# acappemin/Video-to-Audio-and-Piano-RP

Measured on AMD Instinct MI355X. Metric: mel-frames/sec (10s VGGSound shape, 32-step CFM, CFG 2.0), higher is better.
Workload: dtype bf16x3; 1 GPU; BASELINE.json configs[1]: 1 clip(s)/GPU x 750 latent frames x 128 ch, 32-point sway grid = 31 CFG evaluations (62 DiT forwards), T5 context 16 tokens, V2A zero roll; clips_per_gpu=1, global_clips=1, parallelism=clip-sharded x1, 1 all-gather, hipgraph=True, schedule=three streams, side_streams=True, cascade_passes=1

## Files before the change

### video-to-audio-and-piano-rp_amd/csrc/gemm_8phase.hip

```cpp
#include "gemm_common.h"

namespace {

#if defined(V2A_GEMM_PROBE) && defined(V2A_8PH_SKIP)
constexpr int kSkip = V2A_8PH_SKIP;
#else
constexpr int kSkip = 0;
#endif

template <int EPI, typename OutT, int MODE, bool SPLIT>
__global__ __launch_bounds__(512) void gemm_bf16_8ph_kernel(GemmParams p) {
  constexpr bool STAGGER = MODE != 2;
  constexpr int BM = 256, BN = 256, WM = 128, WN = 64, TM = 8, TN = 4;
  constexpr int HALF = 128 * 128;
  constexpr int BUF = 4 * HALF;
  static_assert(!is_glu(EPI) || (TN % 2 == 0), "GEGLU / SWIGLU need value/gate tile pairs");
  extern __shared__ __attribute__((aligned(16))) char smem_raw[];

  const int tid = threadIdx.x;
  const int lane = tid & 63;
  const int wave = __builtin_amdgcn_readfirstlane(tid >> 6);
  const int wr = wave >> 2, wc = wave & 3;
  const int lr = lane & 15, lq = lane >> 4;

  int tm, tn;
  tile_of_block(p, blockIdx.x, tm, tn);
  const int m0 = tm * BM, n0 = tn * BN;

  f32x4 acc[TM][TN];
#pragma unroll
  for (int i = 0; i < TM; ++i)
#pragma unroll
    for (int j = 0; j < TN; ++j) acc[i][j] = f32x4{0.f, 0.f, 0.f, 0.f};

  const int srow = lane >> 3;
  const int schunk = (lane & 7) ^ srow;
  const uint32_t schunk_b = (uint32_t)((SPLIT ? schunk & 3 : schunk) << 4);
  const bool slo = SPLIT && schunk >= 4;
  const int kl = SPLIT ? p.s3_kl : 0;
  uint32_t woff[2][2];
#pragma unroll
  for (int s = 0; s < 2; ++s)
#pragma unroll
    for (int i = 0; i < 2; ++i) {
      const int r = 8 * (wave + 8 * i) + srow;
      const int wrw = n0 + 64 * (r >> 5) + (r & 31) + 32 * s;
      woff[s][i] = (uint32_t)(((int64_t)(wrw < p.N ? wrw : p.N - 1) * p.ldw) * 2) + schunk_b + (slo ? (uint32_t)kl * 2 : 0u);
    }
  const char* wbase = reinterpret_cast<const char*>(p.w);
  constexpr int KS = SPLIT ? 32 : 64;
  constexpr int KSH = SPLIT ? 5 : 6;
  const int nk = p.K / KS;

  const int nseg = p.nseg;
  const int64_t a0 = (int64_t)p.a[0];
  const int64_t da1 = nseg > 1 ? (int64_t)p.a[1] - a0 : 0, da2 = nseg > 2 ? (int64_t)p.a[2] - (int64_t)p.a[1] : 0;
  const int32_t ldb0 = (int32_t)(p.lda[0] * 2);
  const int32_t dl1 = nseg > 1 ? (int32_t)(p.lda[1] * 2) - ldb0 : 0, dl2 = nseg > 2 ? (int32_t)((p.lda[2] - p.lda[1]) * 2) : 0;
  const int kend0 = nseg > 1 ? p.kend[0] : 0x7fffffff, kend1 = nseg > 2 ? p.kend[1] : 0x7fffffff;
  const int dk2 = nseg > 2 ? p.kend[1] - p.kend[0] : 0;
  const int sb0 = SPLIT ? (int)(2 * p.alo[0]) : 0;
  const int dsb1 = SPLIT && nseg > 1 ? (int)(2 * p.alo[1]) - sb0 : 0;
  const int dsb2 = SPLIT && nseg > 2 ? (int)(2 * p.alo[2]) - (sb0 + dsb1) : 0;
  const char* aptr[2];
  int aleft[2] = {0, 0};
  uint32_t aoff[2][2];
  auto a_setup = [&](int s, int kt) {
    const int k0 = kt * KS;
    const bool s1 = k0 >= kend0, s2 = k0 >= kend1;
    const int kbeg = (s1 ? kend0 : 0) + (s2 ? dk2 : 0);
    aptr[s] = reinterpret_cast<const char*>(a0 + (s1 ? da1 : 0) + (s2 ? da2 : 0)) + (int64_t)(k0 - kbeg) * 2;
    const uint32_t ldb = (uint32_t)(ldb0 + (s1 ? dl1 : 0) + (s2 ? dl2 : 0));
    const uint32_t lo = slo ? (uint32_t)(sb0 + (s1 ? dsb1 : 0) + (s2 ? dsb2 : 0)) : 0u;
    const int kstop = min(p.K, s2 ? 0x7fffffff : (s1 ? kend1 : kend0));
    aleft[s] = (kstop - k0) >> KSH;
#pragma unroll
    for (int i = 0; i < 2; ++i) {
      const int r = 8 * (wave + 8 * i) + srow;
      const int ar = m0 + r + ((r >= 64) ? 64 : 0) + 64 * s;
      aoff[s][i] = (uint32_t)(ar < p.M ? ar : p.M - 1) * ldb + schunk_b + lo;
    }
  };
  auto stage_a = [&](int s, int kt, int buf) {
    if (aleft[s] == 0) a_setup(s, kt);
    char* dst = smem_raw + buf * BUF + s * HALF;
#pragma unroll
    for (int i = 0; i < 2; ++i)
      __builtin_amdgcn_global_load_lds((const __attribute__((address_space(1))) void*)(aptr[s] + aoff[s][i]),
                                       (__attribute__((address_space(3))) void*)(dst + (wave + 8 * i) * 1024), 16, 0, 0);
    aptr[s] += 2 * KS;
    --aleft[s];
  };
  const char* wptr = wbase;
  int wleft = 0;
  auto stage_b = [&](int kt, int buf) {
    if (wleft == 0) {
      wptr = wbase + (int64_t)kt * (2 * KS);
      wleft = nk - kt;
    }
#pragma unroll
    for (int s = 0; s < 2; ++s) {
      char* dst = smem_raw + buf * BUF + (2 + s) * HALF;
#pragma unroll
      for (int i = 0; i < 2; ++i) {
        uint32_t wo = woff[s][i];
        asm volatile("" : "+v"(wo));
        __builtin_amdgcn_global_load_lds((const __attribute__((address_space(1))) void*)(wptr + wo),
                                         (__attribute__((address_space(3))) void*)(dst + (wave + 8 * i) * 1024), 16, 0, 0);
      }
    }
    wptr += 2 * KS;
    --wleft;
  };

  const int a_frag_off = (64 * wr + lr) * 128;
  const int b_frag_off = (32 * wc + lr) * 128;
  const int ch0 = ((0 + lq) ^ (lr & 7)) << 4, ch1 = ((4 + lq) ^ (lr & 7)) << 4;
  bf16x8 af[4][2], bf0[2][2], bf1[2][2];
  auto read_a = [&](int s, int buf) {
    const char* base = smem_raw + buf * BUF + s * HALF + a_frag_off;
#pragma unroll
    for (int i = 0; i < 4; ++i) {
      af[i][0] = *reinterpret_cast<const bf16x8*>(base + i * 2048 + ch0);
      af[i][1] = *reinterpret_cast<const bf16x8*>(base + i * 2048 + ch1);
    }
  };
  auto read_b = [&](int s, int buf, bf16x8 (&bf)[2][2]) {
    const char* base = smem_raw + buf * BUF + (2 + s) * HALF + b_frag_off;
#pragma unroll
    for (int j = 0; j < 2; ++j) {
      bf[j][0] = *reinterpret_cast<const bf16x8*>(base + j * 2048 + ch0);
      bf[j][1] = *reinterpret_cast<const bf16x8*>(base + j * 2048 + ch1);
    }
  };
  const int rows_valid = (p.dbg & 512) ? 256 : p.M - m0;
  const bool need0 = wr * 128 < rows_valid, need1 = wr * 128 + 64 < rows_valid;
  auto quadrant = [&](auto sa_c, auto sb_c, const bf16x8 (&bf)[2][2]) {
    constexpr int SA = decltype(sa_c)::value, SB = decltype(sb_c)::value;
    if (!(SA == 0 ? need0 : need1)) return;
    __builtin_amdgcn_s_setprio(1);
    if constexpr (SPLIT) {
#pragma unroll
      for (int t = 0; t < 3; ++t)
#pragma unroll
        for (int i = 0; i < 4; ++i)
#pragma unroll
          for (int j = 0; j < 2; ++j)
            acc[4 * SA + i][2 * SB + j] =
                __builtin_amdgcn_mfma_f32_16x16x32_bf16(af[i][t == 0 ? 1 : 0], bf[j][t == 1 ? 1 : 0], acc[4 * SA + i][2 * SB + j], 0, 0, 0);
    } else {
#pragma unroll
      for (int kk = 0; kk < 2; ++kk)
#pragma unroll
        for (int i = 0; i < 4; ++i)
#pragma unroll
          for (int j = 0; j < 2; ++j)
            acc[4 * SA + i][2 * SB + j] = __builtin_amdgcn_mfma_f32_16x16x32_bf16(af[i][kk], bf[j][kk], acc[4 * SA + i][2 * SB + j], 0, 0, 0);
    }
    __builtin_amdgcn_s_setprio(0);
  };
  using I0 = std::integral_constant<int, 0>;
  using I1 = std::integral_constant<int, 1>;

  float* rs_lds = reinterpret_cast<float*>(smem_raw + 2 * BUF);
  const bool scaled = p.rssq != nullptr && p.vec_epi;
  RowScaleLoad rsl;
  if (scaled && tid < 256) rowscale_load(p, m0 + tid, rsl);
  stage_a(0, 0, 0);
  stage_b(0, 0);
  stage_a(1, 0, 0);
  if (nk > 1) {
    stage_a(0, 1, 1);
    stage_b(1, 1);
    if (scaled && tid < 256) rs_lds[tid] = rowscale_finish(p, rsl);
    asm volatile("s_waitcnt vmcnt(6)" ::: "memory");
  } else {
    if (scaled && tid < 256) rs_lds[tid] = rowscale_finish(p, rsl);
    asm volatile("s_waitcnt vmcnt(0)" ::: "memory");
  }
  __builtin_amdgcn_s_barrier();
  if constexpr (STAGGER) {
    if (wr == 1) __builtin_amdgcn_s_barrier();
  }

  auto ktile = [&](auto buf_c, int t) {
    constexpr int B = decltype(buf_c)::value;
    if (!(kSkip & 4) || t == 0) read_a(0, B);
    if (!(kSkip & 1) || t == 0) read_b(0, B, bf0);
    __builtin_amdgcn_sched_barrier(0);
    __builtin_amdgcn_s_barrier();
    quadrant(I0{}, I0{}, bf0);
    __builtin_amdgcn_sched_barrier(0);
    __builtin_amdgcn_s_barrier();
    if (!(kSkip & 1) || t == 0) read_b(1, B, bf1);
    if (t + 1 < nk && !(kSkip & 8)) stage_a(1, t + 1, B ^ 1);
    __builtin_amdgcn_sched_barrier(0);
    __builtin_amdgcn_s_barrier();
    quadrant(I0{}, I1{}, bf1);
    __builtin_amdgcn_sched_barrier(0);
    __builtin_amdgcn_s_barrier();
    if (!(kSkip & 4) || t == 0) read_a(1, B);
    if (t + 2 < nk && !(kSkip & 8)) stage_a(0, t + 2, B);
    __builtin_amdgcn_sched_barrier(0);
    __builtin_amdgcn_s_barrier();
    quadrant(I1{}, I1{}, bf1);
    __builtin_amdgcn_sched_barrier(0);
    __builtin_amdgcn_s_barrier();
    if (t + 2 < nk) {
      if (!(kSkip & 2)) stage_b(t + 2, B);
      asm volatile("s_waitcnt vmcnt(6)" ::: "memory");
    } else {
      asm volatile("s_waitcnt vmcnt(0)" ::: "memory");
    }
    __builtin_amdgcn_sched_barrier(0);
    __builtin_amdgcn_s_barrier();
    quadrant(I1{}, I0{}, bf0);
    __builtin_amdgcn_sched_barrier(0);
    __builtin_amdgcn_s_barrier();
  };
  for (int t = 0; t < nk; t += 2) {
    ktile(I0{}, t);
    if (t + 1 < nk) ktile(I1{}, t + 1);
  }
  if constexpr (STAGGER) {
    if (wr == 0) __builtin_amdgcn_s_barrier();
  }
  if (p.vec_epi) {
    static_assert(8 * 16 * (WN + 4) * 4 <= 2 * BUF, "epilogue slabs must fit in the ring memory");
    float* tile = reinterpret_cast<float*>(smem_raw) + wave * (16 * (WN + 4));
    EpiPrefetch<EPI, TM, WN, false> pf;
    gemm_epilogue_lds<EPI, OutT, TM, TN, WM, WN, false>(p, acc, tile, m0 + wr * WM, n0 + wc * WN, lane, pf, scaled ? rs_lds + wr * WM : nullptr);
  } else {
    gemm_epilogue<EPI, OutT, TM, TN, WM, WN>(p, acc, m0, n0, wr, wc, lr, lq);
  }
}

template <int EPI, typename OutT>
int launch_8ph(const GemmParams& p_in, hipStream_t s) {
  GemmParams p = p_in;
  v2a_detail::fill_tile_map(p, 256, 256);
  constexpr size_t smem = 2 * 4 * 128 * 128 + 256 * 4;
  const int tiles = ((p.M + 255) / 256) * ((p.N + 255) / 256);
  const int mode = v2a_detail::g_gemm_tuning.use_8phase;
  auto go = [&](auto kern) -> int {
    static std::atomic<uint64_t> lds_set{0};
    if (int rc = v2a_enable_lds(reinterpret_cast<const void*>(kern), smem, lds_set, "v2a_gemm(8-phase)")) return rc;
    hipLaunchKernelGGL(kern, dim3(tiles), dim3(512), smem, s, p);
    return 0;
  };
  int rc;
  if (p.s3_kl != 0) {
    if (mode == 2) rc = go(gemm_bf16_8ph_kernel<EPI, OutT, 2, true>);
    else rc = go(gemm_bf16_8ph_kernel<EPI, OutT, 1, true>);
  } else if constexpr (EPI == V2A_EPI_GELU || EPI == V2A_EPI_SWIGLU) {
    return v2a_fail(V2A_ERR_ARG, "v2a_gemm(8-phase): GELU / SWIGLU need split operands");
  } else {
    if (mode == 2) rc = go(gemm_bf16_8ph_kernel<EPI, OutT, 2, false>);
    else rc = go(gemm_bf16_8ph_kernel<EPI, OutT, 1, false>);
  }
  if (rc) return rc;
  return v2a_check_launch("v2a_gemm(8-phase)");
}

}

int v2a_detail::launch_gemm_8phase(const GemmParams& p, int epilogue, int out_dtype, hipStream_t s) {
  const bool out_f32 = out_dtype == V2A_F32;
  switch (epilogue) {
    case V2A_EPI_STORE:
      return out_f32 ? launch_8ph<V2A_EPI_STORE, float>(p, s) : launch_8ph<V2A_EPI_STORE, bf16_t>(p, s);
    case V2A_EPI_GEGLU:
      return out_f32 ? launch_8ph<V2A_EPI_GEGLU, float>(p, s) : launch_8ph<V2A_EPI_GEGLU, bf16_t>(p, s);
    case V2A_EPI_GELU:
      if (p.s3_kl) return out_f32 ? launch_8ph<V2A_EPI_GELU, float>(p, s) : launch_8ph<V2A_EPI_GELU, bf16_t>(p, s);
      break;
    case V2A_EPI_SWIGLU:
      if (p.s3_kl) return out_f32 ? launch_8ph<V2A_EPI_SWIGLU, float>(p, s) : launch_8ph<V2A_EPI_SWIGLU, bf16_t>(p, s);
      break;
    case V2A_EPI_RESID:
      if (out_f32) return launch_8ph<V2A_EPI_RESID, float>(p, s);
      break;
    case V2A_EPI_GATE_RESID:
      if (out_f32) return launch_8ph<V2A_EPI_GATE_RESID, float>(p, s);
      break;
  }
  return v2a_fail(V2A_ERR_ARG, "v2a_gemm(8-phase): unsupported epilogue %d / out_dtype %d", epilogue, out_dtype);
}
```

### video-to-audio-and-piano-rp_amd/csrc/gemm_common.h

```cpp
#pragma once
#include "v2a_common.h"
#include <stdlib.h>
#include <type_traits>

namespace v2a_detail {

struct GemmParams {
  const void* a[3];
  int64_t lda[3];
  int32_t kend[3];
  int32_t nseg;
  const void* w;
  int64_t ldw;
  const float* bias;
  int32_t M, N, K;
  void* out;
  int64_t ldo;
  bf16_t* out2;
  int64_t ldo2;
  const float* resid;
  int64_t ldr;
  const float* gate;
  const int32_t* step;
  int64_t gss, gbs;
  int32_t rpb;
  const float* rope;
  int32_t rope_cols, rope_pos_off;
  int32_t vec_epi;
  int32_t relu;
  const int32_t* a_rowoff;
  const int32_t* a_koff;
  const int32_t* o_rowoff;
  int32_t krot;
  const float* ngam;
  int64_t ngss, ngbs;
  int32_t nsw_row, nsw_off;
  float* ssq;
  int64_t ssq_ld;
  const float* rssq;
  int64_t rssq_ld;
  int32_t rssq_parts;
  float rnorm;
  int32_t xcd_gm, xcd_gn;
  struct Rect { int32_t m_lo, n_lo, cnt, hm; float rcp; } rect[8];
  int32_t nrect, tiles_m, tiles_n;
  int32_t out2_split, out_split;
  int64_t alo[3];
  int64_t out2_lo;
  int32_t s3_kl;
  int32_t dbg;
};

struct GemmTuning {
  int force_tile;
  int krot;
  int use_8phase;
  int min_tiles_8phase;
  int xcd_grid;
  int dbg;
};
extern GemmTuning g_gemm_tuning;
extern int g_attn_one_group_from;
extern int g_dwconv_rows_per_wave;
extern int g_probe_dbg;
extern int g_dwconv_stream;

int launch_gemm_8phase(const GemmParams& p, int epilogue, int out_dtype, hipStream_t stream);

inline void fill_tile_map(GemmParams& p, int BM, int BN) {
  p.tiles_m = (p.M + BM - 1) / BM;
  p.tiles_n = (p.N + BN - 1) / BN;
  const int gm = p.xcd_gm, gn = p.xcd_gn;
  p.nrect = gm * gn;
  for (int r = 0; r < p.nrect; ++r) {
    const int xm = r / gn, xn = r % gn;
    const int m_lo = xm * p.tiles_m / gm, m_hi = (xm + 1) * p.tiles_m / gm;
    const int n_lo = xn * p.tiles_n / gn, n_hi = (xn + 1) * p.tiles_n / gn;
    const int hm = m_hi - m_lo;
    p.rect[r].m_lo = m_lo;
    p.rect[r].n_lo = n_lo;
    p.rect[r].cnt = hm * (n_hi - n_lo);
    p.rect[r].hm = hm > 0 ? hm : 1;
    p.rect[r].rcp = 1.0f / (float)(hm > 0 ? hm : 1);
  }
}

}

namespace {

using v2a_detail::GemmParams;

__device__ __forceinline__ void tile_of_index(const GemmParams& p, int L, int& tm, int& tn) {
  tm = tn = 0;
#pragma unroll
  for (int r = 0; r < 8; ++r) {
    if (r < p.nrect) {
      const int cnt = p.rect[r].cnt;
      if (L >= 0 && L < cnt) {
        const int hm = p.rect[r].hm;
        int q = (int)((float)L * p.rect[r].rcp);
        int rem = L - q * hm;
        if (rem < 0) { --q; rem += hm; }
        else if (rem >= hm) { ++q; rem -= hm; }
        tn = p.rect[r].n_lo + q;
        tm = p.rect[r].m_lo + rem;
      }
      L -= cnt;
    }
  }
}
__device__ __forceinline__ void tile_of_block(const GemmParams& p, int bid, int& tm, int& tn) {
  const int nwg = p.tiles_m * p.tiles_n;
  const int q = nwg >> 3, r = nwg & 7, xcd = bid & 7;
  const int L = (xcd < r ? xcd * (q + 1) : r * (q + 1) + (xcd - r) * q) + (bid >> 3);
  tile_of_index(p, L, tm, tn);
}

__host__ __device__ constexpr bool is_glu(int epi) { return epi == V2A_EPI_GEGLU || epi == V2A_EPI_SWIGLU; }
template <int EPI, bool FAST> __device__ __forceinline__ float glu_act(float g) {
  if constexpr (EPI == V2A_EPI_SWIGLU) return FAST ? silu_f(g) : silu_exact_f(g);
  else return FAST ? gelu_fast_f(g) : gelu_erf_f(g);
}

template <typename T> struct TileCfg;
template <> struct TileCfg<bf16_t> {
  static constexpr int BK = 64;
  static constexpr int LDS_ROW = 64;
};
template <> struct TileCfg<float> {
  static constexpr int BK = 16;
  static constexpr int LDS_ROW = 20;
};

template <int ROWS, bool SRC_F32> struct StageBf16 {
  static constexpr int N = ROWS / 32;
  bf16x8 r[N];
  __device__ __forceinline__ void load(const void* base, int64_t ld, int row0, int rows_total, int k0, int tid) {
    const int chunk = tid & 7;
#pragma unroll
    for (int i = 0; i < N; ++i) {
      int row = row0 + (tid >> 3) + 32 * i;
      row = row < rows_total ? row : rows_total - 1;
      if constexpr (SRC_F32) {
        const float* p = reinterpret_cast<const float*>(base) + (int64_t)row * ld + k0 + chunk * 8;
        f32x4 lo = *reinterpret_cast<const f32x4*>(p);
        f32x4 hi = *reinterpret_cast<const f32x4*>(p + 4);
        bf16x8 v;
#pragma unroll
        for (int j = 0; j < 4; ++j) {
          v[j] = (bf16_t)lo[j];
          v[4 + j] = (bf16_t)hi[j];
        }
        r[i] = v;
      } else {
        const bf16_t* p = reinterpret_cast<const bf16_t*>(base) + (int64_t)row * ld + k0 + chunk * 8;
        r[i] = *reinterpret_cast<const bf16x8*>(p);
      }
    }
  }
  __device__ __forceinline__ void store(bf16_t* lds, int tid) const {
    const int chunk = tid & 7;
#pragma unroll
    for (int i = 0; i < N; ++i) {
      int row = (tid >> 3) + 32 * i;
      *reinterpret_cast<bf16x8*>(lds + row * 64 + ((chunk ^ (row & 7)) << 3)) = r[i];
    }
  }
};

template <int ROWS> struct StageF32 {
  static constexpr int N = ROWS / 64;
  f32x4 r[N];
  __device__ __forceinline__ void load(const void* base, int64_t ld, int row0, int rows_total, int k0, int tid) {
    const int c4 = tid & 3;
#pragma unroll
    for (int i = 0; i < N; ++i) {
      int row = row0 + (tid >> 2) + 64 * i;
      row = row < rows_total ? row : rows_total - 1;
      const float* p = reinterpret_cast<const float*>(base) + (int64_t)row * ld + k0 + c4 * 4;
      r[i] = *reinterpret_cast<const f32x4*>(p);
    }
  }
  __device__ __forceinline__ void store(float* lds, int tid) const {
    const int c4 = tid & 3;
#pragma unroll
    for (int i = 0; i < N; ++i) {
      int row = (tid >> 2) + 64 * i;
      *reinterpret_cast<f32x4*>(lds + row * 20 + c4 * 4) = r[i];
    }
  }
};

template <typename T, bool A_F32, int ROWS> struct StageSel;
template <bool A_F32, int ROWS> struct StageSel<bf16_t, A_F32, ROWS> { using type = StageBf16<ROWS, A_F32>; };
template <bool A_F32, int ROWS> struct StageSel<float, A_F32, ROWS> { using type = StageF32<ROWS>; };

template <int EPI, typename OutT, int TM, int TN, int WM, int WN>
__device__ __forceinline__ void gemm_epilogue(const GemmParams& p, f32x4 (&acc)[TM][TN], int m0, int n0, int wm, int wn,
                                              int lr, int lq) {
  OutT* out = reinterpret_cast<OutT*>(p.out);
#pragma unroll
  for (int i = 0; i < TM; ++i) {
#pragma unroll
    for (int jj = 0; jj < 4; ++jj) {
      const int m = m0 + wm * WM + i * 16 + lq * 4 + jj;
      if (m >= p.M) continue;
      const float* gvec = nullptr;
      if constexpr (EPI == V2A_EPI_GATE_RESID) gvec = step_vec(p.gate, p.step, p.gss, p.gbs, p.gbs ? m / p.rpb : 0);
      if constexpr (is_glu(EPI)) {
#pragma unroll
        for (int j = 0; j < TN; j += 2) {
          const int n = n0 + wn * WN + j * 16 + lr;
          if (n >= p.N) continue;
          float v = acc[i][j][jj], g = acc[i][j + 1][jj];
          if (p.bias) { v += p.bias[n]; g += p.bias[n + 16]; }
          const int oc = ((n0 + wn * WN) >> 1) + (j >> 1) * 16 + lr;
          const float ge = glu_act<EPI, sizeof(OutT) == 2>(g);
          out[(int64_t)m * p.ldo + oc] = from_f32<OutT>(v * ge);
        }
      } else {
#pragma unroll
        for (int j = 0; j < TN; ++j) {
          const int n = n0 + wn * WN + j * 16 + lr;
          if (n >= p.N) continue;
          float v = acc[i][j][jj];
          if (p.bias) v += p.bias[n];
          if constexpr (EPI == V2A_EPI_SIGMOID) v = sigmoid_f(v);
          if constexpr (EPI == V2A_EPI_GELU) v = gelu_erf_f(v);
          if constexpr (EPI == V2A_EPI_RESID) v += p.resid[(int64_t)m * p.ldr + n];
          if constexpr (EPI == V2A_EPI_GATE_RESID) v = p.resid[(int64_t)m * p.ldr + n] + gvec[n] * v;
          if (p.relu) v = fmaxf(v, 0.f);
          out[(int64_t)m * p.ldo + n] = from_f32<OutT>(v);
          if constexpr (sizeof(OutT) == 4) {
            if (p.out2) p.out2[(int64_t)m * p.ldo2 + n] = (bf16_t)v;
          }
        }
      }
    }
  }
}


template <int EPI, int TM, int WN, bool ON> struct EpiPrefetch {
  static constexpr int LPR = WN / 4, RPI = 64 / LPR, RPS = 16 / RPI;
  static constexpr bool RES = ON && (EPI == V2A_EPI_RESID || EPI == V2A_EPI_GATE_RESID);
  static constexpr bool GATE = ON && EPI == V2A_EPI_GATE_RESID;
  f32x4 rs[RES ? TM : 1][RES ? RPS : 1];
  f32x4 gt[GATE ? TM : 1][GATE ? RPS : 1];
  static constexpr bool SCAT = RES && !GATE;
  int32_t ro[SCAT ? TM : 1][SCAT ? RPS : 1];
  static constexpr bool ROPE = ON && EPI == V2A_EPI_STORE;
  f32x4 cs[ROPE ? TM : 1][ROPE ? RPS : 1];
  __device__ __forceinline__ void load(const GemmParams& p, int m_base, int n_base, int lane) {
    if constexpr (ROPE) {
      const int c4 = (lane % LPR) * 4, r0 = lane / LPR;
      const int n = n_base + c4;
      if (p.rope && n < p.rope_cols) {
#pragma unroll
        for (int i = 0; i < TM; ++i)
#pragma unroll
          for (int q = 0; q < RPS; ++q) {
            int m = m_base + i * 16 + r0 + q * RPI;
            m = m < p.M ? m : p.M - 1;
            const int pos = p.rope_pos_off + m % p.rpb;
            cs[i][q] = *reinterpret_cast<const f32x4*>(p.rope + ((int64_t)pos * 32 + ((n & 63) >> 1)) * 2);
          }
      }
    }
    if constexpr (RES) {
      const int c4 = (lane % LPR) * 4, r0 = lane / LPR;
      const int n = n_base + c4;
      const int M = p.M;
      const bool full = n + 3 < p.N;
      const bool has_res = p.resid != nullptr, has_gate = p.gate != nullptr;
      const float* resid = p.resid + n;
      const int64_t ldr = p.ldr;
      const int32_t* orow = SCAT ? p.o_rowoff : nullptr;
      if constexpr (SCAT) {
        if (orow) {
#pragma unroll
          for (int i = 0; i < TM; ++i)
#pragma unroll
            for (int q = 0; q < RPS; ++q) {
              int m = m_base + i * 16 + r0 + q * RPI;
              m = m < M ? m : M - 1;
              ro[i][q] = orow[m];
            }
        }
      }
#pragma unroll
      for (int i = 0; i < TM; ++i)
#pragma unroll
        for (int q = 0; q < RPS; ++q) {
          const int m = m_base + i * 16 + r0 + q * RPI;
          if (m < M && full) {
            int64_t off = (int64_t)m * ldr;
            if constexpr (SCAT) { if (orow) off = ro[i][q]; }
            rs[i][q] = has_res ? *reinterpret_cast<const f32x4*>(resid + off) : f32x4{0.f, 0.f, 0.f, 0.f};
            if constexpr (GATE) gt[i][q] = has_gate ? *reinterpret_cast<const f32x4*>(step_vec(p.gate, p.step, p.gss, p.gbs, p.gbs ? m / p.rpb : 0) + n) : f32x4{1.f, 1.f, 1.f, 1.f};
          }
        }
    }
  }
};

constexpr int kRowSsqMax = 40;
struct RowScaleLoad {
  f32x4 v[kRowSsqMax / 4];
};
__device__ __forceinline__ void rowscale_load(const GemmParams& p, int m, RowScaleLoad& r) {
  m = m < p.M ? m : p.M - 1;
  const float* q = p.rssq + (int64_t)m * p.rssq_ld;
#pragma unroll
  for (int k = 0; k < kRowSsqMax / 4; ++k) {
    r.v[k] = f32x4{0.f, 0.f, 0.f, 0.f};
    if (4 * k < p.rssq_parts) r.v[k] = *reinterpret_cast<const f32x4*>(q + 4 * k);
  }
}
__device__ __forceinline__ float rowscale_finish(const GemmParams& p, const RowScaleLoad& r) {
  float s = 0.f;
#pragma unroll
  for (int k = 0; k < kRowSsqMax / 4; ++k) s += (r.v[k][0] + r.v[k][1]) + (r.v[k][2] + r.v[k][3]);
  return p.rnorm / fmaxf(sqrtf(s), 1e-12f);
}

__device__ __forceinline__ void rope_rotate4(f32x4& v, const f32x4& cs) {
  const float a0 = v[0], b0 = v[1], a1 = v[2], b1 = v[3];
  v[0] = fmaf(a0, cs[0], -(b0 * cs[1]));
  v[1] = fmaf(b0, cs[0], a0 * cs[1]);
  v[2] = fmaf(a1, cs[2], -(b1 * cs[3]));
  v[3] = fmaf(b1, cs[2], a1 * cs[3]);
}

__device__ __forceinline__ void row_pos(int p0, int d, int rpb, bool multi, int& pos, int& nb) {
  pos = p0 + d;
  nb = 0;
  if (pos >= rpb) { pos -= rpb; nb = 1; }
  if (multi) {
    while (pos >= rpb) { pos -= rpb; ++nb; }
  }
}

template <int EPI, bool PF> constexpr bool epi_pipelined() { return !PF && (EPI == V2A_EPI_STORE || EPI == V2A_EPI_RESID || EPI == V2A_EPI_GATE_RESID); }

template <int EPI, typename OutT, int TM, int TN, int WM, int WN, bool PF, bool ALL>
__device__ __forceinline__ void gemm_epilogue_lds_impl(const GemmParams& p, f32x4 (&acc)[TM][TN], float* tile, int m_base, int n_base, int lane,
                                                       const EpiPrefetch<EPI, TM, WN, PF>& pf, const float* rs_row) {
  constexpr int LD = WN + 4;
  const int lr = lane & 15, lq = lane >> 4;
  OutT* out = reinterpret_cast<OutT*>(p.out);
  const int M = p.M, N = p.N;
  const bool relu = p.relu != 0;
  const int32_t* orow = ALL ? nullptr : p.o_rowoff;
  const int64_t ldo = p.ldo, ldr = p.ldr, ldo2 = p.ldo2;
  bf16_t* out2 = p.out2;
  const float* resid = p.resid;
  const float* bias = p.bias;
  constexpr int LPRX = (is_glu(EPI) ? WN / 2 : WN) / 4;
  constexpr int RPSX = 16 / (64 / LPRX);
  constexpr bool RESF = EPI == V2A_EPI_RESID || EPI == V2A_EPI_GATE_RESID;
  constexpr bool GAMF = RESF && sizeof(OutT) == 4;
  constexpr bool PIPE = epi_pipelined<EPI, PF>();
  static_assert(PIPE || !ALL, "the unpredicated form belongs to the pipeline");
  constexpr int LPRV = WN / 4, RPIV = 64 / LPRV, RPSV = 16 / RPIV;
  const int c4v = (lane % LPRV) * 4, r0v = lane / LPRV;
  const int nv = n_base + c4v;
  const bool fullv = nv + 3 < N;
  const bool scaled = rs_row != nullptr;
  const bool geglu_wide = is_glu(EPI) && sizeof(OutT) == 2 && (WN / 2) % 32 == 0 && ((uintptr_t)p.out & 15) == 0 && (p.ldo & 7) == 0 &&
                          ((p.N >> 1) & 7) == 0 && !(p.dbg & 128);

  f32x4 bb[is_glu(EPI) ? 4 : 1];
#pragma unroll
  for (int k = 0; k < (is_glu(EPI) ? 4 : 1); ++k) bb[k] = f32x4{0.f, 0.f, 0.f, 0.f};
  if constexpr (is_glu(EPI)) {
    if (geglu_wide) {
      const int c8 = (lane % (WN / 16)) * 8;
      const int n = n_base + (c8 >> 4) * 32 + (c8 & 15);
      if (bias && n < N) {
        bb[0] = *reinterpret_cast<const f32x4*>(bias + n);
        bb[1] = *reinterpret_cast<const f32x4*>(bias + n + 4);
        bb[2] = *reinterpret_cast<const f32x4*>(bias + n + 16);
        bb[3] = *reinterpret_cast<const f32x4*>(bias + n + 20);
      }
    } else {
      const int c4 = (lane % (WN / 8)) * 4;
      const int n = n_base + (c4 >> 4) * 32 + (c4 & 15);
      if (bias && n < N) {
        bb[0] = *reinterpret_cast<const f32x4*>(bias + n);
        bb[2] = *reinterpret_cast<const f32x4*>(bias + n + 16);
      }
    }
  } else {
    if (bias && fullv) bb[0] = *reinterpret_cast<const f32x4*>(bias + nv);
  }
  const float* gate_b = nullptr;
  const float* ngam_b = nullptr;
  if constexpr (RESF) {
    const int64_t stepv = p.step ? (int64_t)p.step[0] : 0;
    if (p.gate) gate_b = p.gate + stepv * p.gss;
    if (p.ngam) ngam_b = p.ngam + stepv * p.ngss;
  }
  const int rpb = p.rpb;
  const bool rope_on = PIPE && EPI == V2A_EPI_STORE && p.rope != nullptr && n_base < p.rope_cols;
  static_assert(64 % WN == 0 || EPI != V2A_EPI_STORE || PF, "a wave's columns lie in one 64-column head");
  const bool gate_pb = PIPE && EPI == V2A_EPI_GATE_RESID && gate_b != nullptr && p.gbs != 0;
  const bool gam_on = GAMF && out2 != nullptr && ngam_b != nullptr;
  const bool gam_pb = gam_on && p.ngbs != 0;
  int b0 = 0, p0 = 0;
  bool onebatch = true, twobatch = true;
  if (rope_on || gate_pb || (PIPE && gam_pb)) {
    const int mb = __builtin_amdgcn_readfirstlane(m_base);
    b0 = mb / rpb;
    p0 = mb - b0 * rpb;
    const int last = p0 + ((mb + WM < M ? mb + WM : M) - 1 - mb);
    onebatch = last < rpb;
    twobatch = last < 2 * rpb;
  }
  const int m_sw = m_base - p0 + rpb;
  const bool multi = rpb < WM;
  const bool gate_row = gate_pb && !twobatch, gam_row = gam_pb && !(PIPE && twobatch);
  const bool gate_two = gate_pb && !onebatch && !gate_row, gam_two = PIPE && gam_pb && !onebatch && !gam_row;
  f32x4 gmA = {1.f, 1.f, 1.f, 1.f}, gmB = gmA, gmC = gmA, gmD = gmA, gt1 = gmA, gt2 = gmA;
  if constexpr (GAMF) {
    if (gam_on && !gam_row && fullv && m_base < M) {
      const float* gb = ngam_b + (gam_pb ? (int64_t)b0 * p.ngbs : 0) + nv;
      gmA = *reinterpret_cast<const f32x4*>(gb);
      gmB = *reinterpret_cast<const f32x4*>(gb + p.nsw_off);
      if constexpr (PIPE) {
        if (gam_two) {
          gmC = *reinterpret_cast<const f32x4*>(gb + p.ngbs);
          gmD = *reinterpret_cast<const f32x4*>(gb + p.ngbs + p.nsw_off);
        }
      }
    }
  }
  if constexpr (PIPE && EPI == V2A_EPI_GATE_RESID) {
    if (gate_b && !gate_row && fullv && m_base < M) {
      const float* gp = gate_b + (gate_pb ? (int64_t)b0 * p.gbs : 0) + nv;
      gt1 = *reinterpret_cast<const f32x4*>(gp);
      if (gate_two) gt2 = *reinterpret_cast<const f32x4*>(gp + p.gbs);
    }
  }
  float rsc[PIPE ? 1 : TM][PIPE ? 1 : RPSX];
  if constexpr (!PIPE) {
    if (scaled) {
#pragma unroll
      for (int i = 0; i < TM; ++i)
#pragma unroll
        for (int q = 0; q < RPSX; ++q) rsc[i][q] = rs_row[i * 16 + lane / LPRX + q * (64 / LPRX)];
    }
  }

  f32x4 q_a[PIPE ? 2 : 1][PIPE ? RPSV : 1];
  {
#pragma unroll
    for (int i = -1; i < TM; ++i) {
      if (!ALL && m_base + (i < 0 ? 0 : i) * 16 >= M) break;
      if constexpr (PIPE) {
        if (i + 1 < TM && (ALL || m_base + (i + 1) * 16 < M)) {
#pragma unroll
          for (int q = 0; q < RPSV; ++q) {
            const int m = m_base + (i + 1) * 16 + r0v + q * RPIV;
            const bool ok = ALL || (m < M && fullv);
            if constexpr (EPI == V2A_EPI_STORE) {
              if (rope_on && ok) {
                int pos, nb;
                row_pos(p0, m - m_base, rpb, multi, pos, nb);
                q_a[(i + 1) & 1][q] = *reinterpret_cast<const f32x4*>(p.rope + ((int64_t)(p.rope_pos_off + pos) * 32 + ((nv & 63) >> 1)) * 2);
              }
            }
            if constexpr (RESF) {
              if (ok) {
                int64_t o_res = (int64_t)m * ldr;
                if constexpr (EPI == V2A_EPI_RESID) { if (orow) o_res = orow[m]; }
                q_a[(i + 1) & 1][q] = *reinterpret_cast<const f32x4*>(resid + o_res + nv);
              }
            }
          }
        }
        __builtin_amdgcn_sched_barrier(0);
      }
      if (i < 0) continue;
      if constexpr (PIPE) __builtin_amdgcn_sched_barrier(0);
#pragma unroll
      for (int j = 0; j < TN; ++j)
#pragma unroll
        for (int jj = 0; jj < 4; ++jj) tile[(lq * 4 + jj) * LD + j * 16 + lr] = acc[i][j][jj];
      if (i == 0) {
#pragma unroll
        for (int k = 0; k < (is_glu(EPI) ? 4 : 1); ++k) asm volatile("" : "+v"(bb[k]));
        if constexpr (GAMF) asm volatile("" : "+v"(gmA), "+v"(gmB), "+v"(gmC), "+v"(gmD));
        if constexpr (PIPE && EPI == V2A_EPI_GATE_RESID) asm volatile("" : "+v"(gt1), "+v"(gt2));
      }
      if constexpr (is_glu(EPI) && sizeof(OutT) == 2 && (WN / 2) % 32 == 0) {
        if (geglu_wide) {
          constexpr int OC = WN / 2, LPR = OC / 8, RPI = 64 / LPR;
          static_assert(RPI <= 16, "one slab holds 16 rows");
          const int c8 = (lane % LPR) * 8, r0 = lane / LPR;
          const int lc = (c8 >> 4) * 32 + (c8 & 15);
          const int n = n_base + lc;
#pragma unroll
          for (int q = 0; q < 16 / RPI; ++q) {
            const int r = r0 + q * RPI;
            const int m = m_base + i * 16 + r;
            if (m >= M || n >= N) continue;
            const float rs = scaled ? rs_row[i * 16 + r] : 1.f;
            bf16x8 hi, lo;
#pragma unroll
            for (int h2 = 0; h2 < 2; ++h2) {
              f32x4 v = *reinterpret_cast<const f32x4*>(tile + r * LD + lc + 4 * h2);
              f32x4 g = *reinterpret_cast<const f32x4*>(tile + r * LD + lc + 16 + 4 * h2);
              if (scaled) {
                v *= rs;
                g *= rs;
              }
#pragma unroll
              for (int e = 0; e < 4; ++e) {
                const float o32 = (v[e] + bb[h2][e]) * glu_act<EPI, true>(g[e] + bb[2 + h2][e]);
                hi[4 * h2 + e] = (bf16_t)o32;
                lo[4 * h2 + e] = (bf16_t)(o32 - (float)hi[4 * h2 + e]);
              }
            }
            OutT* dst = out + (int64_t)m * ldo + (n_base >> 1) + c8;
            *reinterpret_cast<bf16x8*>(dst) = hi;
            if (p.out_split) *reinterpret_cast<bf16x8*>(dst + (N >> 1)) = lo;
          }
          continue;
        }
      }
      if constexpr (is_glu(EPI)) {
        constexpr int OC = WN / 2;
        constexpr int LPR = OC / 4;
        constexpr int RPI = 64 / LPR;
        const int c4 = (lane % LPR) * 4, r0 = lane / LPR;
        const int lc = (c4 >> 4) * 32 + (c4 & 15);
        const int n = n_base + lc;
        const f32x4 bv = bb[0], bg = bb[2];
#pragma unroll
        for (int q = 0; q < 16 / RPI; ++q) {
          const int r = r0 + q * RPI;
          const int m = m_base + i * 16 + r;
          if (m >= M || n >= N) continue;
          f32x4 v = *reinterpret_cast<const f32x4*>(tile + r * LD + lc);
          f32x4 g = *reinterpret_cast<const f32x4*>(tile + r * LD + lc + 16);
          if (scaled) {
            v *= rsc[i][q];
            g *= rsc[i][q];
          }
          OutT* dst = out + (int64_t)m * ldo + (n_base >> 1) + c4;
          if constexpr (sizeof(OutT) == 2) {
            if (p.out_split) {
              bf16x4 hi, lo;
#pragma unroll
              for (int e = 0; e < 4; ++e) {
                const float o32 = (v[e] + bv[e]) * glu_act<EPI, true>(g[e] + bg[e]);
                hi[e] = (bf16_t)o32;
                lo[e] = (bf16_t)(o32 - (float)hi[e]);
              }
              *reinterpret_cast<bf16x4*>(dst) = hi;
              *reinterpret_cast<bf16x4*>(dst + (N >> 1)) = lo;
            } else {
              bf16x4 o;
#pragma unroll
              for (int e = 0; e < 4; ++e) o[e] = (bf16_t)((v[e] + bv[e]) * glu_act<EPI, true>(g[e] + bg[e]));
              *reinterpret_cast<bf16x4*>(dst) = o;
            }
          } else {
            f32x4 o;
#pragma unroll
            for (int e = 0; e < 4; ++e) o[e] = (v[e] + bv[e]) * glu_act<EPI, false>(g[e] + bg[e]);
            *reinterpret_cast<f32x4*>(dst) = o;
          }
        }
      } else {
        constexpr int RPI = RPIV;
        const int c4 = c4v, r0 = r0v, n = nv;
        const bool full = fullv;
        const f32x4 bv = bb[0];
#pragma unroll
        for (int q = 0; q < 16 / RPI; ++q) {
          const int r = r0 + q * RPI;
          const int m = m_base + i * 16 + r;
          if (!ALL && (m >= M || !full)) continue;
          int64_t o_out = (int64_t)m * ldo, o_res = (int64_t)m * ldr, o_out2 = (int64_t)m * ldo2;
          if constexpr (EPI == V2A_EPI_STORE || EPI == V2A_EPI_RESID) {
            if (orow) {
              int64_t ro;
              if constexpr (PF && EPI == V2A_EPI_RESID) ro = pf.ro[i][q];
              else ro = orow[m];
              o_out = o_res = o_out2 = ro;
            }
          }
          f32x4 v = *reinterpret_cast<const f32x4*>(tile + r * LD + c4);
          if (scaled) v *= PIPE ? rs_row[i * 16 + r] : rsc[PIPE ? 0 : i][PIPE ? 0 : q];
#pragma unroll
          for (int e = 0; e < 4; ++e) v[e] += bv[e];
          if constexpr (EPI == V2A_EPI_SIGMOID) {
#pragma unroll
            for (int e = 0; e < 4; ++e) v[e] = sigmoid_f(v[e]);
          }
          if constexpr (EPI == V2A_EPI_GELU) {
#pragma unroll
            for (int e = 0; e < 4; ++e) v[e] = sizeof(OutT) == 2 ? gelu_fast_f(v[e]) : gelu_erf_f(v[e]);
          }
          if constexpr (EPI == V2A_EPI_STORE) {
            if constexpr (PF) {
              if (p.rope && n < p.rope_cols) rope_rotate4(v, pf.cs[i][q]);
            } else {
              if (rope_on) rope_rotate4(v, q_a[i & 1][q]);
            }
          }
          if constexpr (RESF) {
            f32x4 rs, gt = {1.f, 1.f, 1.f, 1.f};
            if constexpr (PF) {
              rs = pf.rs[i][q];
              if constexpr (EPI == V2A_EPI_GATE_RESID) gt = pf.gt[i][q];
            } else {
              rs = q_a[i & 1][q];
              if constexpr (EPI == V2A_EPI_GATE_RESID) {
                gt = gate_two && m >= m_sw ? gt2 : gt1;
                if (gate_row) {
                  int pos, nb;
                  row_pos(p0, m - m_base, rpb, true, pos, nb);
                  gt = *reinterpret_cast<const f32x4*>(gate_b + (int64_t)(b0 + nb) * p.gbs + n);
                  asm volatile("" : "+v"(gt));
                }
              }
            }
#pragma unroll
            for (int e = 0; e < 4; ++e) v[e] = rs[e] + gt[e] * v[e];
          }
          if (relu) {
#pragma unroll
            for (int e = 0; e < 4; ++e) v[e] = fmaxf(v[e], 0.f);
          }
          if constexpr (sizeof(OutT) == 2) {
            bf16x4 o;
#pragma unroll
            for (int e = 0; e < 4; ++e) o[e] = (bf16_t)v[e];
            *reinterpret_cast<bf16x4*>(out + o_out + n) = o;
            if constexpr (EPI == V2A_EPI_GELU) {
              if (p.out_split) {
                bf16x4 lo;
#pragma unroll
                for (int e = 0; e < 4; ++e) lo[e] = (bf16_t)(v[e] - (float)o[e]);
                *reinterpret_cast<bf16x4*>(out + o_out + N + n) = lo;
              }
            }
          } else {
            *reinterpret_cast<f32x4*>(out + o_out + n) = v;
            if (out2) {
              f32x4 gm = m >= p.nsw_row ? gmB : gmA;
              if constexpr (GAMF) {
                if constexpr (PIPE) {
                  if (gam_two && m >= m_sw) gm = m >= p.nsw_row ? gmD : gmC;
                }
                if (gam_row) {
                  int pos, nb = 0;
                  if constexpr (PIPE) row_pos(p0, m - m_base, rpb, true, pos, nb);
                  gm = *reinterpret_cast<const f32x4*>(ngam_b + (int64_t)(PIPE ? b0 + nb : m / rpb) * p.ngbs + (m >= p.nsw_row ? p.nsw_off : 0) + n);
                  if constexpr (PIPE) asm volatile("" : "+v"(gm));
                }
              }
              bf16x4 o;
#pragma unroll
              for (int e = 0; e < 4; ++e) o[e] = (bf16_t)(v[e] * gm[e]);
              *reinterpret_cast<bf16x4*>(out2 + o_out2 + n) = o;
              if (p.out2_split) {
                bf16x4 lo;
#pragma unroll
                for (int e = 0; e < 4; ++e) lo[e] = (bf16_t)(v[e] * gm[e] - (float)o[e]);
                *reinterpret_cast<bf16x4*>(out2 + o_out2 + p.out2_lo + n) = lo;
              }
              if (p.ssq) {
                const float ss = octet_sum(v[0] * v[0] + v[1] * v[1] + v[2] * v[2] + v[3] * v[3]);
                if ((lane & 7) == 0) p.ssq[(int64_t)m * p.ssq_ld + (n >> 5)] = ss;
              }
            }
          }
          if constexpr (PIPE) __builtin_amdgcn_sched_barrier(0);
        }
      }
    }
  }
}

template <int EPI, typename OutT, int TM, int TN, int WM, int WN, bool PF>
__device__ __forceinline__ void gemm_epilogue_lds(const GemmParams& p, f32x4 (&acc)[TM][TN], float* tile ,
                                                  int m_base, int n_base, int lane, const EpiPrefetch<EPI, TM, WN, PF>& pf,
                                                  const float* rs_row = nullptr ) {
  if constexpr (epi_pipelined<EPI, PF>()) {
    if (__builtin_amdgcn_readfirstlane((int)(m_base + WM <= p.M && n_base + WN <= p.N)) && p.o_rowoff == nullptr)
      gemm_epilogue_lds_impl<EPI, OutT, TM, TN, WM, WN, PF, true>(p, acc, tile, m_base, n_base, lane, pf, rs_row);
    else
      gemm_epilogue_lds_impl<EPI, OutT, TM, TN, WM, WN, PF, false>(p, acc, tile, m_base, n_base, lane, pf, rs_row);
  } else {
    gemm_epilogue_lds_impl<EPI, OutT, TM, TN, WM, WN, PF, false>(p, acc, tile, m_base, n_base, lane, pf, rs_row);
  }
}

}
```

Before: 3276 mel-frames/s.

## Balance 8-phase GEMM row tiles across M blocks and skip empty MFMA strips

Adds a runtime block height (bm) to the 8-phase GEMM. For small tile counts the M dimension is split evenly across blocks in 32-row multiples instead of fixed 256-row blocks, so the last block is not mostly padding. Each wave-row half covers bm/2 rows, and the fourth 16-row MFMA strip per quadrant is skipped when it holds no valid rows. The epilogue gains a row limit and a flag that drops the last 16-row slab while keeping the fast full-tile path. The change adds a runtime branch inside the MFMA loop and more complex addressing and bounds logic, which risks correctness at boundaries and some scheduling cost.

```diff
diff --git a/video-to-audio-and-piano-rp_amd/csrc/gemm_8phase.hip b/video-to-audio-and-piano-rp_amd/csrc/gemm_8phase.hip
--- a/video-to-audio-and-piano-rp_amd/csrc/gemm_8phase.hip
+++ b/video-to-audio-and-piano-rp_amd/csrc/gemm_8phase.hip
@@ -25,7 +25,9 @@
 
   int tm, tn;
   tile_of_block(p, blockIdx.x, tm, tn);
-  const int m0 = tm * BM, n0 = tn * BN;
+  const int bm = p.bm, hw = bm >> 1;
+  const int m0 = tm * bm, n0 = tn * BN;
+  const int m_end = min(p.M, m0 + bm);
 
   f32x4 acc[TM][TN];
 #pragma unroll
@@ -77,7 +79,7 @@
 #pragma unroll
     for (int i = 0; i < 2; ++i) {
       const int r = 8 * (wave + 8 * i) + srow;
-      const int ar = m0 + r + ((r >= 64) ? 64 : 0) + 64 * s;
+      const int ar = m0 + ((r >= 64) ? hw : 0) + (r & 63) + 64 * s;
       aoff[s][i] = (uint32_t)(ar < p.M ? ar : p.M - 1) * ldb + schunk_b + lo;
     }
   };
@@ -133,29 +135,45 @@
       bf[j][1] = *reinterpret_cast<const bf16x8*>(base + j * 2048 + ch1);
     }
   };
-  const int rows_valid = (p.dbg & 512) ? 256 : p.M - m0;
-  const bool need0 = wr * 128 < rows_valid, need1 = wr * 128 + 64 < rows_valid;
+  const int rows_wr = (p.dbg & 512) ? 128 : max(0, min(hw, m_end - (m0 + wr * hw)));
+  const int nb0 = (min(rows_wr, 64) + 15) >> 4, nb1 = (max(rows_wr - 64, 0) + 15) >> 4;
   auto quadrant = [&](auto sa_c, auto sb_c, const bf16x8 (&bf)[2][2]) {
     constexpr int SA = decltype(sa_c)::value, SB = decltype(sb_c)::value;
-    if (!(SA == 0 ? need0 : need1)) return;
+    const int nb = SA == 0 ? nb0 : nb1;
+    if (nb == 0) return;
     __builtin_amdgcn_s_setprio(1);
     if constexpr (SPLIT) {
 #pragma unroll
       for (int t = 0; t < 3; ++t)
 #pragma unroll
-        for (int i = 0; i < 4; ++i)
+        for (int i = 0; i < 3; ++i)
 #pragma unroll
           for (int j = 0; j < 2; ++j)
             acc[4 * SA + i][2 * SB + j] =
                 __builtin_amdgcn_mfma_f32_16x16x32_bf16(af[i][t == 0 ? 1 : 0], bf[j][t == 1 ? 1 : 0], acc[4 * SA + i][2 * SB + j], 0, 0, 0);
+      if (nb == 4) {
+#pragma unroll
+        for (int t = 0; t < 3; ++t)
+#pragma unroll
+          for (int j = 0; j < 2; ++j)
+            acc[4 * SA + 3][2 * SB + j] =
+                __builtin_amdgcn_mfma_f32_16x16x32_bf16(af[3][t == 0 ? 1 : 0], bf[j][t == 1 ? 1 : 0], acc[4 * SA + 3][2 * SB + j], 0, 0, 0);
+      }
     } else {
 #pragma unroll
       for (int kk = 0; kk < 2; ++kk)
 #pragma unroll
-        for (int i = 0; i < 4; ++i)
+        for (int i = 0; i < 3; ++i)
 #pragma unroll
           for (int j = 0; j < 2; ++j)
             acc[4 * SA + i][2 * SB + j] = __builtin_amdgcn_mfma_f32_16x16x32_bf16(af[i][kk], bf[j][kk], acc[4 * SA + i][2 * SB + j], 0, 0, 0);
+      if (nb == 4) {
+#pragma unroll
+        for (int kk = 0; kk < 2; ++kk)
+#pragma unroll
+          for (int j = 0; j < 2; ++j)
+            acc[4 * SA + 3][2 * SB + j] = __builtin_amdgcn_mfma_f32_16x16x32_bf16(af[3][kk], bf[j][kk], acc[4 * SA + 3][2 * SB + j], 0, 0, 0);
+      }
     }
     __builtin_amdgcn_s_setprio(0);
   };
@@ -229,7 +247,8 @@
     static_assert(8 * 16 * (WN + 4) * 4 <= 2 * BUF, "epilogue slabs must fit in the ring memory");
     float* tile = reinterpret_cast<float*>(smem_raw) + wave * (16 * (WN + 4));
     EpiPrefetch<EPI, TM, WN, false> pf;
-    gemm_epilogue_lds<EPI, OutT, TM, TN, WM, WN, false>(p, acc, tile, m0 + wr * WM, n0 + wc * WN, lane, pf, scaled ? rs_lds + wr * WM : nullptr);
+    gemm_epilogue_lds<EPI, OutT, TM, TN, WM, WN, false>(p, acc, tile, m0 + wr * hw, n0 + wc * WN, lane, pf, scaled ? rs_lds + wr * hw : nullptr,
+                                                         m0 + (wr + 1) * hw);
   } else {
     gemm_epilogue<EPI, OutT, TM, TN, WM, WN>(p, acc, m0, n0, wr, wc, lr, lq);
   }
@@ -241,6 +260,11 @@
   v2a_detail::fill_tile_map(p, 256, 256);
   constexpr size_t smem = 2 * 4 * 128 * 128 + 256 * 4;
   const int tiles = ((p.M + 255) / 256) * ((p.N + 255) / 256);
+  {
+    const int nb = (p.M + 255) / 256;
+    const int even = (((p.M + nb - 1) / nb + 31) / 32) * 32;
+    p.bm = (p.dbg & 1024) || !p.vec_epi || tiles > 256 || even > 256 ? 256 : even;
+  }
   const int mode = v2a_detail::g_gemm_tuning.use_8phase;
   auto go = [&](auto kern) -> int {
     static std::atomic<uint64_t> lds_set{0};
diff --git a/video-to-audio-and-piano-rp_amd/csrc/gemm_common.h b/video-to-audio-and-piano-rp_amd/csrc/gemm_common.h
--- a/video-to-audio-and-piano-rp_amd/csrc/gemm_common.h
+++ b/video-to-audio-and-piano-rp_amd/csrc/gemm_common.h
@@ -48,6 +48,7 @@
   int64_t alo[3];
   int64_t out2_lo;
   int32_t s3_kl;
+  int32_t bm;
   int32_t dbg;
 };
 
@@ -346,11 +347,11 @@
 
 template <int EPI, typename OutT, int TM, int TN, int WM, int WN, bool PF, bool ALL>
 __device__ __forceinline__ void gemm_epilogue_lds_impl(const GemmParams& p, f32x4 (&acc)[TM][TN], float* tile, int m_base, int n_base, int lane,
-                                                       const EpiPrefetch<EPI, TM, WN, PF>& pf, const float* rs_row) {
+                                                       const EpiPrefetch<EPI, TM, WN, PF>& pf, const float* rs_row, int m_lim, bool all_last) {
   constexpr int LD = WN + 4;
   const int lr = lane & 15, lq = lane >> 4;
   OutT* out = reinterpret_cast<OutT*>(p.out);
-  const int M = p.M, N = p.N;
+  const int M = min(p.M, m_lim), N = p.N;
   const bool relu = p.relu != 0;
   const int32_t* orow = ALL ? nullptr : p.o_rowoff;
   const int64_t ldo = p.ldo, ldr = p.ldr, ldo2 = p.ldo2;
@@ -459,7 +460,7 @@
     for (int i = -1; i < TM; ++i) {
       if (!ALL && m_base + (i < 0 ? 0 : i) * 16 >= M) break;
       if constexpr (PIPE) {
-        if (i + 1 < TM && (ALL || m_base + (i + 1) * 16 < M)) {
+        if (i + 1 < TM && (ALL ? (i + 1 < TM - 1 || all_last) : m_base + (i + 1) * 16 < M)) {
 #pragma unroll
           for (int q = 0; q < RPSV; ++q) {
             const int m = m_base + (i + 1) * 16 + r0v + q * RPIV;
@@ -483,6 +484,7 @@
         __builtin_amdgcn_sched_barrier(0);
       }
       if (i < 0) continue;
+      if (ALL && i == TM - 1 && !all_last) continue;
       if constexpr (PIPE) __builtin_amdgcn_sched_barrier(0);
 #pragma unroll
       for (int j = 0; j < TN; ++j)
@@ -690,15 +692,18 @@
 template <int EPI, typename OutT, int TM, int TN, int WM, int WN, bool PF>
 __device__ __forceinline__ void gemm_epilogue_lds(const GemmParams& p, f32x4 (&acc)[TM][TN], float* tile ,
                                                   int m_base, int n_base, int lane, const EpiPrefetch<EPI, TM, WN, PF>& pf,
-                                                  const float* rs_row = nullptr ) {
+                                                  const float* rs_row = nullptr ,
+                                                  int m_lim = 0x7fffffff ) {
   if constexpr (epi_pipelined<EPI, PF>()) {
-    if (__builtin_amdgcn_readfirstlane((int)(m_base + WM <= p.M && n_base + WN <= p.N)) && p.o_rowoff == nullptr)
-      gemm_epilogue_lds_impl<EPI, OutT, TM, TN, WM, WN, PF, true>(p, acc, tile, m_base, n_base, lane, pf, rs_row);
+    const int own = __builtin_amdgcn_readfirstlane(min(m_base + WM, m_lim) - m_base);
+    const bool all_last = own == WM;
+    if (__builtin_amdgcn_readfirstlane((int)((all_last || own == WM - 16) && m_base + own <= p.M && n_base + WN <= p.N)) && p.o_rowoff == nullptr)
+      gemm_epilogue_lds_impl<EPI, OutT, TM, TN, WM, WN, PF, true>(p, acc, tile, m_base, n_base, lane, pf, rs_row, m_lim, all_last);
     else
-      gemm_epilogue_lds_impl<EPI, OutT, TM, TN, WM, WN, PF, false>(p, acc, tile, m_base, n_base, lane, pf, rs_row);
+      gemm_epilogue_lds_impl<EPI, OutT, TM, TN, WM, WN, PF, false>(p, acc, tile, m_base, n_base, lane, pf, rs_row, m_lim, true);
   } else {
-    gemm_epilogue_lds_impl<EPI, OutT, TM, TN, WM, WN, PF, false>(p, acc, tile, m_base, n_base, lane, pf, rs_row);
-  }
-}
-
-}
+    gemm_epilogue_lds_impl<EPI, OutT, TM, TN, WM, WN, PF, false>(p, acc, tile, m_base, n_base, lane, pf, rs_row, m_lim, true);
+  }
+}
+
+}
```

Result: no change. 3248 mel-frames/s (-0.9%).
